# BadgerTechnologies/navigation

Hardware: AMD Instinct MI355X
Metric: scored trajectories/sec (whole node) + costmap inflation cells/sec, 400x400 map (higher is better)
Workload: dtype f64

## Files before the change

### navigation_amd/csrc/planner_bfs_rows.hip

```cpp
#include "planner_common.h"

namespace navgpu {

#ifdef NAVGPU_BFS_STATS
__device__ unsigned long long g_bfs_stats[16];
#define BFS_STAMP(v) const unsigned long long v = __builtin_amdgcn_s_memtime()
#define BFS_ACC(i, x) bst[i] += (x)
#else
#define BFS_STAMP(v)
#define BFS_ACC(i, x)
#endif
#ifndef NAVGPU_ROWS_RECORD_PAD
#define NAVGPU_ROWS_RECORD_PAD 4
#endif
constexpr uint32_t kRowsRecordPad = NAVGPU_ROWS_RECORD_PAD;
template <int W>
__host__ __device__ inline size_t bfs_rows_lds_words(uint32_t nx, uint32_t ny) {
  constexpr uint32_t Wp = (W + 3) & ~3u;
  const uint32_t nw = bfs_rows_waves(ny);
  return (((size_t)nw * kRowsPerWave * ((nx + 31) >> 5) + 3) & ~(size_t)3) + (size_t)kCareRows * kCareWords + (size_t)(nw + 2) * 2 * kRowsHalo * (2 * Wp + kRowsRecordPad);
}
__device__ __forceinline__ void rowsGroup4(const int g, const uint32_t aw, uint32_t& nz, uint32_t& lo, uint32_t& hi, uint32_t* __restrict__ b,
                                           uint32_t* __restrict__ f, const uint32_t L, const uint32_t R, uint32_t& p) {
  uint32_t u0, u1, u2, u3, t0, t1, t2, t3, st;
// ... 234 lines not shown
      BFS_ACC(7, aw != 0 ? 1 : 0);
      BFS_ACC(8, __builtin_popcount(aw));
      if (aw != 0) {
        uint32_t nz = 0, lo = 0, hi = 0;
        uint32_t p[2];
        const uint32_t zero = 0;
#pragma unroll
        for (int q = 0; q < NG; ++q)
          rowsGroup4(q, aw, nz, lo, hi, &blocked[4 * q], &fr[4 * q], q > 0 ? p[(q + 1) & 1] : zero, q + 1 < NG ? fr[q + 1 < NG ? 4 * q + 4 : 0] : zero,
                     p[q & 1]);
        BFS_STAMP(ts2);
        BFS_ACC(1, ts2 - ts1);
        if (wave_in_box && (nz & region_groups) != 0) {
#pragma unroll
          for (int q = 0; q < NG; ++q) {
            if (((nz & region_groups) >> q) & 1u) {
#pragma unroll
              for (int c = 0; c < 4; ++c) {
                const int j = 4 * q + c;
                if (j < W && j >= w0 && j <= w1) {
#ifndef NAVGPU_BFS_X_NOSTORE
                  if (row_in_box && fr[j < W ? j : 0] != 0) storeCells(j, fr[j < W ? j : 0], level + 1);
#endif
                }
              }
            }
          }
        }
        BFS_STAMP(ts3);
        BFS_ACC(2, ts3 - ts2);
        any_blk |= nz;
        a_own = (nz | (lo >> 1) | (hi << 1)) & gmask;
      }
      ++level;
    }
    BFS_STAMP(ts4);
    const uint32_t slot = xch % 3u;
    if (pub_top || pub_bot) {
#pragma unroll
      for (int q = 0; q < WP; q += 4) {
        *reinterpret_cast<uint4*>(edge + pub_wr + q) = make_uint4(fr[q], fr[q + 1], fr[q + 2], fr[q + 3]);
        *reinterpret_cast<uint4*>(edge + pub_wr + WP + q) = make_uint4(blocked[q], blocked[q + 1], blocked[q + 2], blocked[q + 3]);
      }
    }
    if (any_blk) s_flag[slot] = 1;
    if (wave_in_box) {
      uint32_t open_any = 0;
      const uint32_t rr = (uint32_t)(row_i - by0);
#pragma unroll
      for (int j = 0; j < W; ++j) {
        if (j >= w0 && j <= w1) {
          const uint32_t cw_i = (uint32_t)(j - w0);
          if (row_in_box) {
            const uint32_t care = (care_ok != 0 && cw_i < (uint32_t)kCareWords && rr < (uint32_t)kCareRows) ? care_l[rr * kCareWords + cw_i] : (care_ok ? 0u : 0xFFFFFFFFu);
            const int c_lo = max(bx0 - j * 32, 0), c_hi = min(bx1 - j * 32, 31);
            const uint32_t open = (~blocked[j] & care) | fr[j];
            if (c_hi >= c_lo) open_any |= open & (0xFFFFFFFFu >> (31 - c_hi)) & (0xFFFFFFFFu << c_lo);
          }
        }
      }
      if (open_any != 0) s_open[slot] = 1;
    }
    if (tid == 0) {
      s_flag[(xch + 1) % 3u] = 0;
      s_open[(xch + 1) % 3u] = 0;
    }
    BFS_STAMP(ts5);
    BFS_ACC(3, ts5 - ts4);
    __syncthreads();
    done = !s_flag[slot] || !s_open[slot];
    if (!done) {
      if ((halo_top || halo_bot) && real) {
#pragma unroll
        for (int q = 0; q < WP; q += 4) {
          const uint4 v = *reinterpret_cast<const uint4*>(edge + halo_rd + q);
          const uint4 b = *reinterpret_cast<const uint4*>(edge + halo_rd + WP + q);
          fr[q] = v.x;
          fr[q + 1] = v.y;
          fr[q + 2] = v.z;
          fr[q + 3] = v.w;
          blocked[q] = b.x;
          blocked[q + 1] = b.y;
          blocked[q + 2] = b.z;
          blocked[q + 3] = b.w;
        }
      }
      a_own = activity();
      __syncthreads();
    }
    ++xch;
    any_blk = 0;
    BFS_STAMP(ts6);
    BFS_ACC(4, ts6 - ts5);
  }
#ifdef NAVGPU_BFS_STATS
  if (lane == 0)
    for (int k = 0; k < 9; ++k) atomicAdd(&g_bfs_stats[k], bst[k]);
#endif
  if (pl.bfs_trace && tid == 0) pl.bfs_trace[(size_t)item * 8 + 3] = wall_clock64();

  __syncthreads();
  {
    uint32_t ex[WP], fb[WP];
#pragma unroll
    for (int j = 0; j < WP; ++j) {
      const bool in = owner && (uint32_t)j < Wr;
      fb[j] = in ? (freew[row * Wr + j] & ((uint32_t)j + 1 == Wr ? last_mask : 0xFFFFFFFFu)) : 0u;
      ex[j] = in ? ((blocked[j] & fb[j]) | seedm[row * Wr + j]) : 0u;
    }
    if (pub_top || pub_bot) {
#pragma unroll
      for (int j = 0; j < WP; ++j) edge[pub_wr + j] = ex[j];
    }
    __syncthreads();
    if ((halo_top || halo_bot) && real) {
#pragma unroll
      for (int j = 0; j < WP; ++j) ex[j] = edge[halo_rd + j];
    }
    if (wave_in_box) {
#pragma unroll
      for (int j = 0; j < W; ++j) {
        if (j >= w0 && j <= w1) {
          const uint32_t fc = ex[j];
          const uint32_t lw = j > 0 ? ex[j > 0 ? j - 1 : 0] : 0u, rw = j + 1 < WP ? ex[j + 1 < WP ? j + 1 : 0] : 0u;
          const uint32_t nbr = __builtin_amdgcn_alignbit(fc, lw, 31) | __builtin_amdgcn_alignbit(rw, fc, 1) | fromLaneBelow(fc) | fromLaneAbove(fc);
          const uint32_t cm = (uint32_t)j + 1 == Wr ? last_mask : ((uint32_t)j < Wr ? 0xFFFFFFFFu : 0u);
          const uint32_t touched = nbr & ~fb[j] & ~fc & cm;
          if (row_in_box) {
            storeCells(j, touched, N_obst);
            storeCells(j, ~fc & ~touched & cm, N_unreach);
          }
        }
      }
    }
  }
  if (pl.bfs_trace && tid == 0) {
    pl.bfs_trace[(size_t)item * 8 + 6] = wall_clock64();
    pl.bfs_trace[(size_t)item * 8 + 1] = wall_clock64() | ((unsigned long long)level << 48);
  }
  if (tid == 0 && pl.bfs_grids == 3) pl.bfs_levels[(size_t)inst * 3 + which] = level;
}
template <int W>
__global__ __launch_bounds__(1024, 6) void k_bfs_rows(PlannerDev pl, uint32_t first, uint32_t count, uint32_t* next_item, const uint32_t* order) {
  __shared__ uint32_t s_item;
  const uint32_t total = count * pl.bfs_grids;
  for (;;) {
    if (threadIdx.x == 0) s_item = atomicAdd(next_item, 1u);
    __syncthreads();
    const uint32_t slot = s_item;
    if (slot >= total) break;
    const uint32_t item = order ? order[slot] : slot;
    const uint32_t g = item / count;
    bfsRowsGrid<W>(pl, first + (item - g * count), (int)pl.bfs_grids - 1 - (int)g, item);
    __syncthreads();
  }
}
constexpr int kRows2HaloLanes = 4;
constexpr int kRows2Levels = 2 * kRows2HaloLanes;
constexpr int kRows2PerWave = 2 * (64 - 2 * kRows2HaloLanes);
constexpr int kRows2Words = 32;
__host__ __device__ inline uint32_t bfs_rows2_waves(uint32_t ny) { return (ny + kRows2PerWave - 1) / kRows2PerWave; }
__host__ __device__ inline size_t bfs_rows2_lds_words(uint32_t ny) {
  return (size_t)kCareRows * kCareWords + (size_t)(bfs_rows2_waves(ny) + 2) * 2 * kRows2HaloLanes * 4 * kRows2Words;
}
template <int G>
__device__ __forceinline__ void rows2Group(const uint32_t aw, uint32_t& nz, uint32_t& lo, uint32_t& hi, uint32_t* __restrict__ bA, uint32_t* __restrict__ bB,
                                           uint32_t* __restrict__ fA, uint32_t* __restrict__ fB, uint32_t& pA, uint32_t& pB, const uint32_t rA,
                                           const uint32_t rB) {
  uint32_t u0, u1, u2, u3, v0, v1, v2, v3, h0, h1, h2, h3, st;
#define NAVGPU_ROWS2_HEAD_FIRST                \
  "s_bitcmp1_b32 %[aw], %[g]\n\t"              \
  "s_cbranch_scc0 1f\n\t"                      \
  "v_lshlrev_b32 %[u0], 1, %[fA0]\n\t"         \
  "v_lshlrev_b32 %[v0], 1, %[fB0]\n\t"
#define NAVGPU_ROWS2_HEAD_NEXT                 \
  "s_bitcmp1_b32 %[aw], %[g]\n\t"              \
  "s_cbranch_scc0 1f\n\t"                      \
  "s_bitcmp1_b32 %[aw], %[gp]\n\t"             \
  "s_cbranch_scc1 3f\n\t"                      \
  "v_lshlrev_b32 %[u0], 1, %[fA0]\n\t"         \
  "v_lshlrev_b32 %[v0], 1, %[fB0]\n\t"         \
  "s_branch 4f\n\t"                            \
  "3:\n\t"                                     \
  "v_alignbit_b32 %[u0], %[fA0], %[pA], 31\n\t" \
  "v_alignbit_b32 %[v0], %[fB0], %[pB], 31\n\t" \
  "4:\n\t"
#define NAVGPU_ROWS2_BODY(HEAD)                                                                        \
  asm volatile(                                                                                        \
      HEAD                                                                                             \
      "v_alignbit_b32 %[u1], %[fA1], %[fA0], 31\n\t"                                                   \
      "v_alignbit_b32 %[u2], %[fA2], %[fA1], 31\n\t"                                                   \
      "v_alignbit_b32 %[u3], %[fA3], %[fA2], 31\n\t"                                                   \
      "v_alignbit_b32 %[v1], %[fB1], %[fB0], 31\n\t"                                                   \
      "v_alignbit_b32 %[v2], %[fB2], %[fB1], 31\n\t"                                                   \
      "v_alignbit_b32 %[v3], %[fB3], %[fB2], 31\n\t"                                                   \
      "v_mov_b32 %[pA], %[fA3]\n\t"                                                                    \
      "v_mov_b32 %[pB], %[fB3]\n\t"                                                                    \
      "v_alignbit_b32 %[h0], %[fA1], %[fA0], 1\n\t"                                                    \
      "v_alignbit_b32 %[h1], %[fA2], %[fA1], 1\n\t"                                                    \
      "v_alignbit_b32 %[h2], %[fA3], %[fA2], 1\n\t"                                                    \
      "v_alignbit_b32 %[h3], %[rA], %[fA3], 1\n\t"                                                     \
      "v_or_b32_dpp %[u0], %[fB0], %[u0] wave_shr:1 row_mask:0xf bank_mask:0xf bound_ctrl:1\n\t"       \
      "v_or_b32_dpp %[u1], %[fB1], %[u1] wave_shr:1 row_mask:0xf bank_mask:0xf bound_ctrl:1\n\t"       \
      "v_or_b32_dpp %[u2], %[fB2], %[u2] wave_shr:1 row_mask:0xf bank_mask:0xf bound_ctrl:1\n\t"       \
      "v_or_b32_dpp %[u3], %[fB3], %[u3] wave_shr:1 row_mask:0xf bank_mask:0xf bound_ctrl:1\n\t"       \
      "v_or3_b32 %[u0], %[u0], %[h0], %[fB0]\n\t"                                                      \
      "v_or3_b32 %[u1], %[u1], %[h1], %[fB1]\n\t"                                                      \
      "v_or3_b32 %[u2], %[u2], %[h2], %[fB2]\n\t"                                                      \
      "v_or3_b32 %[u3], %[u3], %[h3], %[fB3]\n\t"                                                      \
      "v_alignbit_b32 %[h0], %[fB1], %[fB0], 1\n\t"                                                    \
      "v_alignbit_b32 %[h1], %[fB2], %[fB1], 1\n\t"                                                    \
      "v_alignbit_b32 %[h2], %[fB3], %[fB2], 1\n\t"                                                    \
      "v_alignbit_b32 %[h3], %[rB], %[fB3], 1\n\t"                                                     \
      "v_or_b32_dpp %[v0], %[fA0], %[v0] wave_shl:1 row_mask:0xf bank_mask:0xf bound_ctrl:1\n\t"       \
      "v_or_b32_dpp %[v1], %[fA1], %[v1] wave_shl:1 row_mask:0xf bank_mask:0xf bound_ctrl:1\n\t"       \
      "v_or_b32_dpp %[v2], %[fA2], %[v2] wave_shl:1 row_mask:0xf bank_mask:0xf bound_ctrl:1\n\t"       \
      "v_or_b32_dpp %[v3], %[fA3], %[v3] wave_shl:1 row_mask:0xf bank_mask:0xf bound_ctrl:1\n\t"       \
      "v_or3_b32 %[v0], %[v0], %[h0], %[fA0]\n\t"                                                      \
      "v_or3_b32 %[v1], %[v1], %[h1], %[fA1]\n\t"                                                      \
      "v_or3_b32 %[v2], %[v2], %[h2], %[fA2]\n\t"                                                      \
      "v_or3_b32 %[v3], %[v3], %[h3], %[fA3]\n\t"                                                      \
      "v_bitop3_b32 %[fA0], %[u0], %[bA0], %[u0] bitop3:0x30\n\t"                                      \
      "v_bitop3_b32 %[fA1], %[u1], %[bA1], %[u1] bitop3:0x30\n\t"                                      \
      "v_bitop3_b32 %[fA2], %[u2], %[bA2], %[u2] bitop3:0x30\n\t"                                      \
      "v_bitop3_b32 %[fA3], %[u3], %[bA3], %[u3] bitop3:0x30\n\t"                                      \
      "v_bitop3_b32 %[fB0], %[v0], %[bB0], %[v0] bitop3:0x30\n\t"                                      \
      "v_bitop3_b32 %[fB1], %[v1], %[bB1], %[v1] bitop3:0x30\n\t"                                      \
      "v_bitop3_b32 %[fB2], %[v2], %[bB2], %[v2] bitop3:0x30\n\t"                                      \
      "v_bitop3_b32 %[fB3], %[v3], %[bB3], %[v3] bitop3:0x30\n\t"                                      \
      "v_or_b32_e32 %[bA0], %[bA0], %[u0]\n\t"                                                         \
      "v_or_b32_e32 %[bA1], %[bA1], %[u1]\n\t"                                                         \
      "v_or_b32_e32 %[bA2], %[bA2], %[u2]\n\t"                                                         \
      "v_or_b32_e32 %[bA3], %[bA3], %[u3]\n\t"                                                         \
      "v_or_b32_e32 %[bB0], %[bB0], %[v0]\n\t"                                                         \
      "v_or_b32_e32 %[bB1], %[bB1], %[v1]\n\t"                                                         \
      "v_or_b32_e32 %[bB2], %[bB2], %[v2]\n\t"                                                         \
      "v_or_b32_e32 %[bB3], %[bB3], %[v3]\n\t"                                                         \
      "v_or_b32_e32 %[h0], %[fA0], %[fB0]\n\t"                                                         \
      "v_or_b32_e32 %[h3], %[fA3], %[fB3]\n\t"                                                         \
      "v_or3_b32 %[h1], %[fA1], %[fA2], %[fB1]\n\t"                                                    \
      "v_or3_b32 %[h2], %[h0], %[h3], %[fB2]\n\t"                                                      \
      "v_or_b32_e32 %[h1], %[h1], %[h2]\n\t"                                                           \
      "v_cmp_ne_u32_e32 vcc, 0, %[h1]\n\t"                                                             \
      "s_cbranch_vccz 1f\n\t"                                                                          \
      "s_bitset1_b32 %[nz], %[g]\n\t"                                                                  \
      "v_cmp_ne_u32_e32 vcc, 0, %[h0]\n\t"                                                             \
      "s_cbranch_vccz 3f\n\t"                                                                          \
      "s_bitset1_b32 %[lo], %[g]\n\t"                                                                  \
      "3:\n\t"                                                                                         \
      "v_cmp_ne_u32_e32 vcc, 0, %[h3]\n\t"                                                             \
      "s_cbranch_vccz 1f\n\t"                                                                          \
      "s_bitset1_b32 %[hi], %[g]\n\t"                                                                  \
      "1:\n\t"                                                                                         \
      : [bA0] "+v"(bA[0]), [bA1] "+v"(bA[1]), [bA2] "+v"(bA[2]), [bA3] "+v"(bA[3]), [bB0] "+v"(bB[0]), [bB1] "+v"(bB[1]), [bB2] "+v"(bB[2]),  \
        [bB3] "+v"(bB[3]), [fA0] "+v"(fA[0]), [fA1] "+v"(fA[1]), [fA2] "+v"(fA[2]), [fA3] "+v"(fA[3]), [fB0] "+v"(fB[0]), [fB1] "+v"(fB[1]),   \
        [fB2] "+v"(fB[2]), [fB3] "+v"(fB[3]), [pA] "+v"(pA), [pB] "+v"(pB), [nz] "+s"(nz), [lo] "+s"(lo), [hi] "+s"(hi), [u0] "=&v"(u0),       \
        [u1] "=&v"(u1), [u2] "=&v"(u2), [u3] "=&v"(u3), [v0] "=&v"(v0), [v1] "=&v"(v1), [v2] "=&v"(v2), [v3] "=&v"(v3), [h0] "=&v"(h0),        \
        [h1] "=&v"(h1), [h2] "=&v"(h2), [h3] "=&v"(h3), [st] "=&s"(st)                                                                         \
      : [aw] "s"(aw), [g] "n"(G), [gp] "n"(G > 0 ? G - 1 : 0), [rA] "v"(rA), [rB] "v"(rB)                                                      \
      : "vcc", "scc")
  if constexpr (G == 0) NAVGPU_ROWS2_BODY(NAVGPU_ROWS2_HEAD_FIRST);
  else NAVGPU_ROWS2_BODY(NAVGPU_ROWS2_HEAD_NEXT);
#undef NAVGPU_ROWS2_BODY
#undef NAVGPU_ROWS2_HEAD_FIRST
#undef NAVGPU_ROWS2_HEAD_NEXT
}
template <int G>
__device__ __forceinline__ void rows2Level(const uint32_t aw, uint32_t& nz, uint32_t& lo, uint32_t& hi, uint32_t* __restrict__ blA, uint32_t* __restrict__ blB,
                                           uint32_t* __restrict__ frA, uint32_t* __restrict__ frB, uint32_t& pA, uint32_t& pB, const uint32_t zero) {
  constexpr int NG = kRows2Words / 4;
  if constexpr (G < NG) {
    rows2Group<G>(aw, nz, lo, hi, blA + 4 * G, blB + 4 * G, frA + 4 * G, frB + 4 * G, pA, pB, G + 1 < NG ? frA[G + 1 < NG ? 4 * G + 4 : 0] : zero,
                  G + 1 < NG ? frB[G + 1 < NG ? 4 * G + 4 : 0] : zero);
    rows2Level<G + 1>(aw, nz, lo, hi, blA, blB, frA, frB, pA, pB, zero);
  }
}
__device__ __forceinline__ void bfsRows2Grid(const PlannerDev& pl, const uint32_t inst, const int which, const uint32_t item, uint32_t* seedw) {
  constexpr int W = kRows2Words, NG = W / 4, D = kRows2Levels, HL = kRows2HaloLanes;
  int bx0 = 0, bx1 = -1, by0 = 0, by1 = -1, care_ok = 0;
  if (pl.bfs_bounded) {
    const int4 bb = reinterpret_cast<const int4*>(pl.bfs_box)[2 * inst];
    bx0 = __builtin_amdgcn_readfirstlane(bb.x);
    bx1 = __builtin_amdgcn_readfirstlane(bb.y);
    by0 = __builtin_amdgcn_readfirstlane(bb.z);
    by1 = __builtin_amdgcn_readfirstlane(bb.w);
    care_ok = __builtin_amdgcn_readfirstlane(pl.bfs_box[8 * inst + 4]);
  }
  if (!(bx1 >= bx0 && by1 >= by0)) {
    bx0 = 0;
    by0 = 0;
    bx1 = (int)pl.nx - 1;
    by1 = (int)pl.ny - 1;
    care_ok = 0;
  }
  extern __shared__ __align__(16) uint32_t sm[];
  __shared__ uint32_t s_wave[16];
  __shared__ uint32_t s_flag[3];
  __shared__ uint32_t s_open[3];
  uint32_t tid_ = threadIdx.x, nx_ = pl.nx, ny_ = pl.ny;
  asm volatile("" : "+v"(tid_), "+s"(nx_), "+s"(ny_));
  const uint32_t tid = tid_;
  if (pl.bfs_trace && tid == 0) pl.bfs_trace[(size_t)item * 8] = wall_clock64();
  const Geom g = geomOf(pl, inst);
  const uint32_t nx = nx_, ny = ny_, Wr = (nx + 31) >> 5;
  const uint32_t nw = blockDim.x >> 6;
  const uint32_t lane = tid & 63u, wave_id = tid >> 6;
// ... 174 lines not shown
    if (any_blk) s_flag[slot] = 1;
    if (wave_in_box) {
      uint32_t open_any = 0;
      const uint32_t rrA = (uint32_t)(rowA_i - by0), rrB = (uint32_t)(rowB_i - by0);
#pragma unroll
      for (int j = 0; j < W; ++j) {
        if (j >= w0 && j <= w1) {
          const uint32_t cw_i = (uint32_t)(j - w0);
          const int c_lo = max(bx0 - j * 32, 0), c_hi = min(bx1 - j * 32, 31);
          const uint32_t cm = c_hi >= c_lo ? ((0xFFFFFFFFu >> (31 - c_hi)) & (0xFFFFFFFFu << c_lo)) : 0u;
          if (inA) {
            const uint32_t care = (care_ok != 0 && cw_i < (uint32_t)kCareWords && rrA < (uint32_t)kCareRows) ? care_l[rrA * kCareWords + cw_i] : (care_ok ? 0u : 0xFFFFFFFFu);
            open_any |= ((~blA[j] & care) | frA[j]) & cm;
          }
          if (inB) {
            const uint32_t care = (care_ok != 0 && cw_i < (uint32_t)kCareWords && rrB < (uint32_t)kCareRows) ? care_l[rrB * kCareWords + cw_i] : (care_ok ? 0u : 0xFFFFFFFFu);
            open_any |= ((~blB[j] & care) | frB[j]) & cm;
          }
        }
      }
      if (open_any != 0) s_open[slot] = 1;
    }
    if (tid == 0) {
      s_flag[(xch + 1) % 3u] = 0;
      s_open[(xch + 1) % 3u] = 0;
    }
    BFS_STAMP(ts5);
    BFS_ACC(3, ts5 - ts4);
    __syncthreads();
    done = !s_flag[slot] || !s_open[slot];
    if (!done) {
      if (halo_top || halo_bot) {
#pragma unroll
        for (int q = 0; q < W; q += 4) {
          if (realA) {
            unquad(*reinterpret_cast<const uint4*>(edge + halo_rd + q), frA + q);
            unquad(*reinterpret_cast<const uint4*>(edge + halo_rd + W + q), blA + q);
          }
          if (realB) {
            unquad(*reinterpret_cast<const uint4*>(edge + halo_rd + 2 * W + q), frB + q);
            unquad(*reinterpret_cast<const uint4*>(edge + halo_rd + 3 * W + q), blB + q);
          }
        }
      }
      a_own = activity();
      __syncthreads();
    }
    ++xch;
    any_blk = 0;
    BFS_STAMP(ts6);
    BFS_ACC(4, ts6 - ts5);
  }
#ifdef NAVGPU_BFS_STATS
  if (lane == 0)
    for (int k = 0; k < 9; ++k) atomicAdd(&g_bfs_stats[k], bst[k]);
#endif
  if (pl.bfs_trace && tid == 0) pl.bfs_trace[(size_t)item * 8 + 3] = wall_clock64();

  __syncthreads();
  {
#pragma unroll
    for (int q = 0; q < NG; ++q) {
      const uint4 sA = ownerA ? rowWords(seedw, rowA, q) : make_uint4(0, 0, 0, 0), sB = ownerB ? rowWords(seedw, rowB, q) : make_uint4(0, 0, 0, 0);
      const uint4 fA = ownerA ? rowWords(freew, rowA, q) : make_uint4(0, 0, 0, 0), fB = ownerB ? rowWords(freew, rowB, q) : make_uint4(0, 0, 0, 0);
      const uint32_t sa[4] = {sA.x, sA.y, sA.z, sA.w}, sb[4] = {sB.x, sB.y, sB.z, sB.w}, fa[4] = {fA.x, fA.y, fA.z, fA.w}, fb[4] = {fB.x, fB.y, fB.z, fB.w};
#pragma unroll
      for (int c = 0; c < 4; ++c) {
        const int j = 4 * q + c;
        const bool in = (uint32_t)j < Wr;
        blA[j] = (in && ownerA) ? ((blA[j] & fa[c] & colMask(j)) | sa[c]) : 0u;
        blB[j] = (in && ownerB) ? ((blB[j] & fb[c] & colMask(j)) | sb[c]) : 0u;
      }
    }
    if (lane == (uint32_t)HL || lane == 63u - HL) {
      const bool top = lane == (uint32_t)HL;
      uint32_t* rec = edge + ((wave_id + 1) * 2 + (top ? 0u : 1u)) * HL * 4 * W;
#pragma unroll
      for (int j = 0; j < W; ++j) rec[j] = top ? blA[j] : blB[j];
    }
    __syncthreads();
    if (lane == (uint32_t)HL - 1u && realB) {
      const uint32_t* rec = edge + (wave_id * 2 + 1) * HL * 4 * W;
#pragma unroll
      for (int j = 0; j < W; ++j) blB[j] = rec[j];
    }
    if (lane == 64u - HL && realA) {
      const uint32_t* rec = edge + ((wave_id + 2) * 2) * HL * 4 * W;
#pragma unroll
      for (int j = 0; j < W; ++j) blA[j] = rec[j];
    }
    if (wave_in_box) {
#pragma unroll
      for (int j = 0; j < W; ++j) {
        if (j >= w0 && j <= w1) {
          const uint32_t cm = (uint32_t)j + 1 == Wr ? last_mask : ((uint32_t)j < Wr ? 0xFFFFFFFFu : 0u);
          const uint32_t eA = blA[j], eB = blB[j];
          const uint32_t lA = j > 0 ? blA[j > 0 ? j - 1 : 0] : 0u, rA = j + 1 < W ? blA[j + 1 < W ? j + 1 : 0] : 0u;
          const uint32_t lB = j > 0 ? blB[j > 0 ? j - 1 : 0] : 0u, rB = j + 1 < W ? blB[j + 1 < W ? j + 1 : 0] : 0u;
          const uint32_t upA = fromLaneBelow(eB), dnB = fromLaneAbove(eA);
          if (inA) {
            const uint32_t nbr = __builtin_amdgcn_alignbit(eA, lA, 31) | __builtin_amdgcn_alignbit(rA, eA, 1) | upA | eB;
            const uint32_t fb = freew[rowA * Wr + j] & cm;
            const uint32_t touched = nbr & ~fb & ~eA & cm;
            storeCells(rowA, j, touched, N_obst);
            storeCells(rowA, j, ~eA & ~touched & cm, N_unreach);
          }
          if (inB) {
            const uint32_t nbr = __builtin_amdgcn_alignbit(eB, lB, 31) | __builtin_amdgcn_alignbit(rB, eB, 1) | eA | dnB;
            const uint32_t fb = freew[rowB * Wr + j] & cm;
            const uint32_t touched = nbr & ~fb & ~eB & cm;
            storeCells(rowB, j, touched, N_obst);
            storeCells(rowB, j, ~eB & ~touched & cm, N_unreach);
          }
        }
      }
    }
  }
  if (pl.bfs_trace && tid == 0) {
    pl.bfs_trace[(size_t)item * 8 + 6] = wall_clock64();
    pl.bfs_trace[(size_t)item * 8 + 1] = wall_clock64() | ((unsigned long long)level << 48);
  }
  if (tid == 0 && pl.bfs_grids == 3) pl.bfs_levels[(size_t)inst * 3 + which] = level;
}
__global__ __launch_bounds__(768, 3) void k_bfs_rows2(PlannerDev pl, uint32_t first, uint32_t count, uint32_t* next_item, const uint32_t* order, uint32_t* scratch) {
  __shared__ uint32_t s_item;
  const uint32_t total = count * pl.bfs_grids;
  uint32_t* seedw = scratch + (size_t)blockIdx.x * pl.ny * ((pl.nx + 31) >> 5);
  for (;;) {
    if (threadIdx.x == 0) s_item = atomicAdd(next_item, 1u);
    __syncthreads();
    const uint32_t slot = s_item;
    if (slot >= total) break;
    const uint32_t item = order ? order[slot] : slot;
    const uint32_t g = item / count;
    bfsRows2Grid(pl, first + (item - g * count), (int)pl.bfs_grids - 1 - (int)g, item, seedw);
    __syncthreads();
  }
}
static int bfs_rows_words(uint32_t nx, uint32_t ny) {
  if (NAVGPU_DEBUG_ENV("NAVGPU_DEBUG_BFS_NO_ROWS")) return 0;
  const uint32_t Wr = (nx + 31) / 32;
  if (bfs_rows_waves(ny) > 16) return 0;
  return Wr <= 7 ? 7 : (Wr <= 13 ? 13 : (Wr <= 20 ? 20 : 0));
}
bool bfs_rows_fits(uint32_t nx, uint32_t ny) { return bfs_rows_words(nx, ny) != 0; }
template <int W>
static void launch_bfs_rows_w(const PlannerDev& pl, uint32_t first, uint32_t count, hipStream_t s, const uint32_t* order) {
  const uint32_t nw = bfs_rows_waves(pl.ny);
  const size_t lds = bfs_rows_lds_words<W>(pl.nx, pl.ny) * 4;
  if (lds > 48 * 1024) hipFuncSetAttribute((const void*)k_bfs_rows<W>, hipFuncAttributeMaxDynamicSharedMemorySize, (int)lds);
  const uint32_t per_cu = std::max<uint32_t>(1u, std::min<uint32_t>(std::min<uint32_t>(24u / nw, (uint32_t)((156u * 1024u) / (lds + 1024))), 4u));
  hipLaunchKernelGGL(k_bfs_rows<W>, dim3(std::min(count * pl.bfs_grids, per_cu * bfs_cu_count())), dim3(nw * 64), lds, s, pl, first, count, pl.bfs_next_item + 1, order);
}
bool launch_bfs_rows(const PlannerDev& pl, uint32_t first, uint32_t count, hipStream_t s, const uint32_t* order) {
  switch (bfs_rows_words(pl.nx, pl.ny)) {
    case 7: launch_bfs_rows_w<7>(pl, first, count, s, order); return true;
    case 13: launch_bfs_rows_w<13>(pl, first, count, s, order); return true;
    case 20: launch_bfs_rows_w<20>(pl, first, count, s, order); return true;
    default: return false;
  }
}
bool launch_bfs_rows2(const PlannerDev& pl, uint32_t first, uint32_t count, hipStream_t s, const uint32_t* order) {
  if (NAVGPU_DEBUG_ENV("NAVGPU_DEBUG_BFS_NO_ROWS")) return false;
  if ((pl.nx + 31) / 32 > (uint32_t)kRows2Words || bfs_rows2_waves(pl.ny) > 12) return false;
  const size_t lds2 = bfs_rows2_lds_words(pl.ny) * 4;
  if (lds2 > 48 * 1024) hipFuncSetAttribute((const void*)k_bfs_rows2, hipFuncAttributeMaxDynamicSharedMemorySize, (int)lds2);
  hipLaunchKernelGGL(k_bfs_rows2, dim3(std::min(count * pl.bfs_grids, bfs_cu_count())), dim3(bfs_rows2_waves(pl.ny) * 64), lds2, s, pl, first, count, pl.bfs_next_item, order, pl.bfs_scratch);
  return true;
}

#ifdef NAVGPU_BFS_STATS
extern "C" int navgpu_debug_bfs_stats(unsigned long long* out16, int reset) {
  if (out16) hipMemcpyFromSymbol(out16, HIP_SYMBOL(g_bfs_stats), sizeof(unsigned long long) * 16);
  if (reset) {
    unsigned long long z[16] = {0};
    hipMemcpyToSymbol(HIP_SYMBOL(g_bfs_stats), z, sizeof(z));
  }
  return 0;
}
#endif

}
```

Baseline: 5.641 billion.

## Add column-split row BFS variant using two waves per row block

New measurement: 5.399 billion. 0.957x the previous value.

```diff
diff --git a/navigation_amd/csrc/planner_bfs_rows.hip b/navigation_amd/csrc/planner_bfs_rows.hip
--- a/navigation_amd/csrc/planner_bfs_rows.hip
+++ b/navigation_amd/csrc/planner_bfs_rows.hip
@@ -410,6 +410,343 @@
     const uint32_t item = order ? order[slot] : slot;
     const uint32_t g = item / count;
     bfsRowsGrid<W>(pl, first + (item - g * count), (int)pl.bfs_grids - 1 - (int)g, item);
+    __syncthreads();
+  }
+}
+constexpr int kRowsSplitCut = 7;
+constexpr int kRowsSplitWords = 8;
+#ifndef NAVGPU_ROWS_SPLIT_HALO
+#define NAVGPU_ROWS_SPLIT_HALO 7
+#endif
+constexpr int kRowsSplitHalo = NAVGPU_ROWS_SPLIT_HALO;
+constexpr int kRowsSplitPerWave = 64 - 2 * kRowsSplitHalo;
+constexpr uint32_t kRowsSplitRecord = 2 * kRowsSplitWords + kRowsRecordPad;
+__host__ __device__ inline uint32_t bfs_rows_split_blocks(uint32_t ny) { return (ny + kRowsSplitPerWave - 1) / kRowsSplitPerWave; }
+__host__ __device__ inline size_t bfs_rows_split_lds_words(uint32_t nx, uint32_t ny) {
+  const uint32_t nb = bfs_rows_split_blocks(ny);
+  return (((size_t)nb * kRowsSplitPerWave * ((nx + 31) >> 5) + 3) & ~(size_t)3) + (size_t)kCareRows * kCareWords +
+         (size_t)(nb + 2) * 2 * 2 * kRowsSplitHalo * kRowsSplitRecord + (size_t)nb * 2 * 64 * 2;
+}
+template <int W>
+__device__ __forceinline__ void bfsRowsSplitGrid(const PlannerDev& pl, const uint32_t inst, const int which, const uint32_t item) {
+  constexpr int CUT = kRowsSplitCut, WP = kRowsSplitWords, NG = WP / 4, D = kRowsSplitHalo, RPW = kRowsSplitPerWave;
+  static_assert(W > CUT && CUT + 1 <= WP && W - CUT + 1 <= WP, "either half and its halo word fit the lane's words");
+  int bx0 = 0, bx1 = -1, by0 = 0, by1 = -1, care_ok = 0;
+  if (pl.bfs_bounded) {
+    const int4 bb = reinterpret_cast<const int4*>(pl.bfs_box)[2 * inst];
+    bx0 = __builtin_amdgcn_readfirstlane(bb.x);
+    bx1 = __builtin_amdgcn_readfirstlane(bb.y);
+    by0 = __builtin_amdgcn_readfirstlane(bb.z);
+    by1 = __builtin_amdgcn_readfirstlane(bb.w);
+    care_ok = __builtin_amdgcn_readfirstlane(pl.bfs_box[8 * inst + 4]);
+  }
+  if (!(bx1 >= bx0 && by1 >= by0)) {
+    bx0 = 0;
+    by0 = 0;
+    bx1 = (int)pl.nx - 1;
+    by1 = (int)pl.ny - 1;
+    care_ok = 0;
+  }
+  extern __shared__ __align__(16) uint32_t sm[];
+  __shared__ uint32_t s_wave[16];
+  __shared__ uint32_t s_flag[3];
+  __shared__ uint32_t s_open[3];
+  uint32_t tid_ = threadIdx.x, nx_ = pl.nx, ny_ = pl.ny;
+  asm volatile("" : "+v"(tid_), "+s"(nx_), "+s"(ny_));
+  const uint32_t tid = tid_;
+  if (pl.bfs_trace && tid == 0) pl.bfs_trace[(size_t)item * 8] = wall_clock64();
+  const Geom g = geomOf(pl, inst);
+  const uint32_t nx = nx_, ny = ny_, Wr = (nx + 31) >> 5;
+  const uint32_t nb = blockDim.x >> 7;
+  const uint32_t lane = tid & 63u, wave_id = (uint32_t)__builtin_amdgcn_readfirstlane((int)(tid >> 6));
+  const uint32_t rb = wave_id >> 1, half = wave_id & 1u;
+  const int off = half ? CUT - 1 : 0;
+  const int row_i = (int)(rb * RPW + lane) - D;
+  const bool real = row_i >= 0 && row_i < (int)ny;
+  const bool owner = real && lane >= (uint32_t)D && lane < 64u - D;
+  const uint32_t row = real ? (uint32_t)row_i : 0u;
+  const uint32_t rows_p = nb * RPW;
+  const uint32_t seed_words = (rows_p * Wr + 3u) & ~3u;
+  constexpr uint32_t RS = kRowsSplitRecord;
+  uint32_t* seedm = sm;
+  uint32_t* care_l = sm + seed_words;
+  uint32_t* edge = care_l + kCareRows * kCareWords;
+  const uint32_t edge_words = (nb + 2) * 2 * 2 * D * RS;
+  uint32_t* cut = edge + edge_words;
+  const uint32_t cut_words = nb * 2 * 64 * 2;
+  const uint8_t* master = pl.master + (size_t)inst * pl.cells_padded;
+  const uint32_t* freew = bfsFreeBitmap(pl, which, inst, ny * Wr);
+  uint32_t* dist = (which == 0 ? pl.path : (which == 1 ? pl.goal : pl.goal_front)) + (size_t)inst * pl.cells;
+  const uint32_t N_obst = pl.cells, N_unreach = pl.cells + 1;
+  const uint32_t last_mask = (nx & 31) ? ((1u << (nx & 31)) - 1u) : 0xFFFFFFFFu;
+  const bool aligned4 = (nx & 3) == 0;
+
+  for (uint32_t i = tid; i < seed_words + kCareRows * kCareWords + edge_words + cut_words; i += blockDim.x) sm[i] = 0;
+  if (tid < 3) s_flag[tid] = s_open[tid] = 0;
+  __syncthreads();
+  if (pl.bfs_trace && tid == 0) pl.bfs_trace[(size_t)item * 8 + 4] = wall_clock64();
+  if (care_ok) {
+    const uint32_t* care = pl.bfs_care + (size_t)inst * kCareRows * kCareWords;
+    for (uint32_t i = tid; i < (uint32_t)(kCareRows * kCareWords); i += blockDim.x) care_l[i] = care[i];
+  }
+  rowsPlanSeeds(pl, inst, which, g, master, nx, tid, s_wave, [&](uint32_t mx, uint32_t my) {
+    atomicOr(&seedm[my * Wr + (mx >> 5)], 1u << (mx & 31));
+  });
+  __syncthreads();
+  if (pl.bfs_trace && tid == 0) pl.bfs_trace[(size_t)item * 8 + 5] = wall_clock64();
+
+  const uint32_t* freer = freew + row * Wr + off;
+  const uint32_t* seedr = seedm + row * Wr + off;
+  uint32_t blocked[WP], fr[WP];
+#pragma unroll
+  for (int j = 0; j < WP; ++j) {
+    blocked[j] = 0xFFFFFFFFu;
+    fr[j] = 0;
+    if (real && (uint32_t)(j + off) < Wr) {
+      fr[j] = seedr[j];
+      blocked[j] = ~(freer[j] & ((uint32_t)(j + off) + 1 == Wr ? last_mask : 0xFFFFFFFFu)) | fr[j];
+    }
+  }
+  const int lw0 = max(bx0 >> 5, half ? CUT : 0) - off, lw1 = min(min(bx1 >> 5, half ? W - 1 : CUT - 1), (int)Wr - 1) - off;
+  const bool wave_in_box = (int)(rb * RPW) <= by1 && (int)((rb + 1) * RPW) > by0 && lw1 >= lw0;
+  const bool row_in_box = owner && row_i >= by0 && row_i <= by1;
+  const int cw0 = off - (bx0 >> 5);
+  uint32_t region_groups = 0;
+  for (int jr = lw0; jr <= lw1; ++jr) region_groups |= 1u << (jr >> 2);
+  uint32_t* drow = dist + (size_t)row * nx + off * 32;
+  auto storeCells = [&](int j, uint32_t cells, uint32_t value) {
+    uint32_t* dw = drow + j * 32;
+    if (aligned4) {
+      uint32_t full = cells & (cells >> 1) & (cells >> 2) & (cells >> 3) & 0x11111111u;
+      cells &= ~(full * 15u);
+      const uint4 v4 = make_uint4(value, value, value, value);
+      while (full) {
+        const uint32_t bpos = (uint32_t)__ffs(full) - 1u;
+        *reinterpret_cast<uint4*>(dw + bpos) = v4;
+        full &= full - 1;
+      }
+    }
+    while (cells) {
+      const uint32_t bpos = (uint32_t)__ffs(cells) - 1u;
+      dw[bpos] = value;
+      cells &= cells - 1;
+    }
+  };
+  auto vrec = [&](uint32_t slot, uint32_t h, uint32_t bottom) { return ((slot * 2 + h) * 2 + bottom) * D; };
+  const bool pub_top = lane >= (uint32_t)D && lane < 2u * D, pub_bot = lane >= 64u - 2 * D && lane < 64u - D;
+  const uint32_t pub_wr = (vrec(rb + 1, half, pub_top ? 0u : 1u) + (pub_top ? lane - D : lane - (64u - 2 * D))) * RS;
+  const bool halo_top = lane < (uint32_t)D, halo_bot = lane >= 64u - D;
+  const uint32_t halo_row = halo_top ? lane : lane - (64u - D);
+  const uint32_t halo_rd = (vrec(halo_top ? rb : rb + 2, half, halo_top ? 1u : 0u) + halo_row) * RS;
+  const uint32_t corner_rd = (vrec(halo_top ? rb : rb + 2, half ^ 1u, halo_top ? 1u : 0u) + halo_row) * RS + (half ? CUT - 1 : 1);
+  const uint32_t cut_wr = (wave_id * 64 + lane) * 2, cut_rd = ((wave_id ^ 1u) * 64 + lane) * 2;
+  constexpr uint32_t gmask = (1u << NG) - 1u;
+
+  auto activity = [&]() -> uint32_t {
+    uint32_t nz = 0, lo = 0, hi = 0;
+#pragma unroll
+    for (int q = 0; q < NG; ++q) {
+      const uint32_t t = fr[4 * q] | fr[4 * q + 1] | fr[4 * q + 2] | fr[4 * q + 3];
+      if (__builtin_amdgcn_ballot_w64(t != 0) != 0) {
+        nz |= 1u << q;
+        if (__builtin_amdgcn_ballot_w64(fr[4 * q] != 0) != 0) lo |= 1u << q;
+        if (__builtin_amdgcn_ballot_w64(fr[4 * q + 3] != 0) != 0) hi |= 1u << q;
+      }
+    }
+    return (nz | (lo >> 1) | (hi << 1)) & gmask;
+  };
+  if (wave_in_box) {
+    uint32_t seed_dist = 0;
+    asm volatile("" : "+s"(seed_dist));
+#pragma unroll
+    for (int j = 0; j < WP; ++j)
+      if (j >= lw0 && j <= lw1 && row_in_box) storeCells(j, fr[j], seed_dist);
+  }
+  uint32_t a_own = activity();
+  uint32_t level = 0, xch = 0, any_blk = 0;
+  if (pl.bfs_trace && tid == 0) pl.bfs_trace[(size_t)item * 8 + 2] = wall_clock64();
+  bool done = false;
+#ifdef NAVGPU_BFS_STATS
+  unsigned long long bst[9] = {0, 0, 0, 0, 0, 0, 0, 0, 0};
+#endif
+  while (!done) {
+    for (int k = 0; k < D; ++k) {
+      BFS_STAMP(ts1);
+      BFS_ACC(5, 1);
+      const uint32_t aw = __builtin_amdgcn_readfirstlane(a_own);
+      BFS_ACC(7, aw != 0 ? 1 : 0);
+      BFS_ACC(8, __builtin_popcount(aw));
+      if (aw != 0) {
+        uint32_t nz = 0, lo = 0, hi = 0;
+        uint32_t p[2];
+        const uint32_t zero = 0;
+        rowsGroup4(0, aw, nz, lo, hi, &blocked[0], &fr[0], zero, fr[4], p[0]);
+        rowsGroup4(1, aw, nz, lo, hi, &blocked[4], &fr[4], p[0], zero, p[1]);
+        BFS_STAMP(ts2);
+        BFS_ACC(1, ts2 - ts1);
+        if (wave_in_box && (nz & region_groups) != 0) {
+#pragma unroll
+          for (int q = 0; q < NG; ++q) {
+            if (((nz & region_groups) >> q) & 1u) {
+#pragma unroll
+              for (int c = 0; c < 4; ++c) {
+                const int j = 4 * q + c;
+                if (j >= lw0 && j <= lw1) {
+                  if (row_in_box && fr[j] != 0) storeCells(j, fr[j], level + 1);
+                }
+              }
+            }
+          }
+        }
+        BFS_STAMP(ts3);
+        BFS_ACC(2, ts3 - ts2);
+        any_blk |= nz;
+        a_own = (nz | (lo >> 1) | (hi << 1)) & gmask;
+      }
+      ++level;
+    }
+    BFS_STAMP(ts4);
+    const uint32_t slot = xch % 3u;
+    if (pub_top || pub_bot) {
+#pragma unroll
+      for (int q = 0; q < WP; q += 4) {
+        *reinterpret_cast<uint4*>(edge + pub_wr + q) = make_uint4(fr[q], fr[q + 1], fr[q + 2], fr[q + 3]);
+        *reinterpret_cast<uint4*>(edge + pub_wr + WP + q) = make_uint4(blocked[q], blocked[q + 1], blocked[q + 2], blocked[q + 3]);
+      }
+    }
+    *reinterpret_cast<uint2*>(cut + cut_wr) = half ? make_uint2(fr[1], blocked[1]) : make_uint2(fr[CUT - 1], blocked[CUT - 1]);
+    if (any_blk) s_flag[slot] = 1;
+    if (wave_in_box) {
+      uint32_t open_any = 0;
+      const uint32_t rr = (uint32_t)(row_i - by0);
+#pragma unroll
+      for (int j = 0; j < WP; ++j) {
+        if (j >= lw0 && j <= lw1) {
+          const uint32_t cw_i = (uint32_t)(j + cw0);
+          if (row_in_box) {
+            const uint32_t care = (care_ok != 0 && cw_i < (uint32_t)kCareWords && rr < (uint32_t)kCareRows) ? care_l[rr * kCareWords + cw_i] : (care_ok ? 0u : 0xFFFFFFFFu);
+            const int c_lo = max(bx0 - (j + off) * 32, 0), c_hi = min(bx1 - (j + off) * 32, 31);
+            const uint32_t open = (~blocked[j] & care) | fr[j];
+            if (c_hi >= c_lo) open_any |= open & (0xFFFFFFFFu >> (31 - c_hi)) & (0xFFFFFFFFu << c_lo);
+          }
+        }
+      }
+      if (open_any != 0) s_open[slot] = 1;
+    }
+    if (tid == 0) {
+      s_flag[(xch + 1) % 3u] = 0;
+      s_open[(xch + 1) % 3u] = 0;
+    }
+    BFS_STAMP(ts5);
+    BFS_ACC(3, ts5 - ts4);
+    __syncthreads();
+    done = !s_flag[slot] || !s_open[slot];
+    if (!done) {
+      uint32_t hf, hb;
+      if (halo_top || halo_bot) {
+        if (real) {
+#pragma unroll
+          for (int q = 0; q < WP; q += 4) {
+            const uint4 v = *reinterpret_cast<const uint4*>(edge + halo_rd + q);
+            const uint4 b = *reinterpret_cast<const uint4*>(edge + halo_rd + WP + q);
+            fr[q] = v.x;
+            fr[q + 1] = v.y;
+            fr[q + 2] = v.z;
+            fr[q + 3] = v.w;
+            blocked[q] = b.x;
+            blocked[q + 1] = b.y;
+            blocked[q + 2] = b.z;
+            blocked[q + 3] = b.w;
+          }
+        }
+        hf = edge[corner_rd];
+        hb = edge[corner_rd + WP];
+      } else {
+        const uint2 c = *reinterpret_cast<const uint2*>(cut + cut_rd);
+        hf = c.x;
+        hb = c.y;
+      }
+      if (real) {
+        if (half) {
+          fr[0] = hf;
+          blocked[0] = hb;
+        } else {
+          fr[CUT] = hf;
+          blocked[CUT] = hb;
+        }
+      }
+      a_own = activity();
+      __syncthreads();
+    }
+    ++xch;
+    any_blk = 0;
+    BFS_STAMP(ts6);
+    BFS_ACC(4, ts6 - ts5);
+  }
+#ifdef NAVGPU_BFS_STATS
+  if (lane == 0)
+    for (int k = 0; k < 9; ++k) atomicAdd(&g_bfs_stats[k], bst[k]);
+#endif
+  if (pl.bfs_trace && tid == 0) pl.bfs_trace[(size_t)item * 8 + 3] = wall_clock64();
+
+  __syncthreads();
+  {
+    uint32_t ex[WP], fb[WP];
+#pragma unroll
+    for (int j = 0; j < WP; ++j) {
+      const bool in = owner && j >= (half ? 1 : 0) && j < (half ? WP : CUT) && (uint32_t)(j + off) < Wr;
+      fb[j] = in ? (freer[j] & ((uint32_t)(j + off) + 1 == Wr ? last_mask : 0xFFFFFFFFu)) : 0u;
+      ex[j] = in ? ((blocked[j] & fb[j]) | seedr[j]) : 0u;
+    }
+    if (pub_top || pub_bot) {
+#pragma unroll
+      for (int j = 0; j < WP; ++j) edge[pub_wr + j] = ex[j];
+    }
+    cut[cut_wr] = half ? ex[1] : ex[CUT - 1];
+    __syncthreads();
+    if ((halo_top || halo_bot) && real) {
+#pragma unroll
+      for (int j = 0; j < WP; ++j) ex[j] = edge[halo_rd + j];
+    } else if (!(halo_top || halo_bot)) {
+      const uint32_t c = cut[cut_rd];
+      if (half) ex[0] = c;
+      else ex[CUT] = c;
+    }
+    if (wave_in_box) {
+#pragma unroll
+      for (int j = 0; j < WP; ++j) {
+        if (j >= lw0 && j <= lw1) {
+          const uint32_t fc = ex[j];
+          const uint32_t lw = j > 0 ? ex[j > 0 ? j - 1 : 0] : 0u, rw = j + 1 < WP ? ex[j + 1 < WP ? j + 1 : 0] : 0u;
+          const uint32_t nbr = __builtin_amdgcn_alignbit(fc, lw, 31) | __builtin_amdgcn_alignbit(rw, fc, 1) | fromLaneBelow(fc) | fromLaneAbove(fc);
+          const uint32_t cm = (uint32_t)(j + off) + 1 == Wr ? last_mask : 0xFFFFFFFFu;
+          const uint32_t touched = nbr & ~fb[j] & ~fc & cm;
+          if (row_in_box) {
+            storeCells(j, touched, N_obst);
+            storeCells(j, ~fc & ~touched & cm, N_unreach);
+          }
+        }
+      }
+    }
+  }
+  if (pl.bfs_trace && tid == 0) {
+    pl.bfs_trace[(size_t)item * 8 + 6] = wall_clock64();
+    pl.bfs_trace[(size_t)item * 8 + 1] = wall_clock64() | ((unsigned long long)level << 48);
+  }
+  if (tid == 0 && pl.bfs_grids == 3) pl.bfs_levels[(size_t)inst * 3 + which] = level;
+}
+template <int W>
+__global__ __launch_bounds__(1024, 8) void k_bfs_rows_split(PlannerDev pl, uint32_t first, uint32_t count, uint32_t* next_item, const uint32_t* order) {
+  __shared__ uint32_t s_item;
+  const uint32_t total = count * pl.bfs_grids;
+  for (;;) {
+    if (threadIdx.x == 0) s_item = atomicAdd(next_item, 1u);
+    __syncthreads();
+    const uint32_t slot = s_item;
+    if (slot >= total) break;
+    const uint32_t item = order ? order[slot] : slot;
+    const uint32_t g = item / count;
+    bfsRowsSplitGrid<W>(pl, first + (item - g * count), (int)pl.bfs_grids - 1 - (int)g, item);
     __syncthreads();
   }
 }
@@ -890,10 +1227,27 @@
   const uint32_t per_cu = std::max<uint32_t>(1u, std::min<uint32_t>(std::min<uint32_t>(24u / nw, (uint32_t)((156u * 1024u) / (lds + 1024))), 4u));
   hipLaunchKernelGGL(k_bfs_rows<W>, dim3(std::min(count * pl.bfs_grids, per_cu * bfs_cu_count())), dim3(nw * 64), lds, s, pl, first, count, pl.bfs_next_item + 1, order);
 }
+constexpr uint32_t kRowsSplitSlotShareNum = 1, kRowsSplitSlotShareDen = 2;
+static bool bfs_rows_split_takes(const PlannerDev& pl, uint32_t count) {
+  const uint32_t Wr = (pl.nx + 31) / 32, nb = bfs_rows_split_blocks(pl.ny);
+  if (Wr <= (uint32_t)kRowsSplitCut || nb > 8) return false;
+  if (const char* e = NAVGPU_DEBUG_ENV("NAVGPU_DEBUG_BFS_SPLIT")) return e[0] != '0';
+  return (uint64_t)count * pl.bfs_grids * 2 * nb * kRowsSplitSlotShareDen <= (uint64_t)bfs_cu_count() * 32 * kRowsSplitSlotShareNum;
+}
+static void launch_bfs_rows_split13(const PlannerDev& pl, uint32_t first, uint32_t count, hipStream_t s, const uint32_t* order) {
+  const uint32_t nb = bfs_rows_split_blocks(pl.ny);
+  const size_t lds = bfs_rows_split_lds_words(pl.nx, pl.ny) * 4;
+  if (lds > 48 * 1024) hipFuncSetAttribute((const void*)k_bfs_rows_split<13>, hipFuncAttributeMaxDynamicSharedMemorySize, (int)lds);
+  const uint32_t per_cu = std::max<uint32_t>(1u, std::min<uint32_t>(std::min<uint32_t>(16u / nb, (uint32_t)((156u * 1024u) / (lds + 1024))), 4u));
+  hipLaunchKernelGGL(k_bfs_rows_split<13>, dim3(std::min(count * pl.bfs_grids, per_cu * bfs_cu_count())), dim3(nb * 128), lds, s, pl, first, count, pl.bfs_next_item + 1, order);
+}
 bool launch_bfs_rows(const PlannerDev& pl, uint32_t first, uint32_t count, hipStream_t s, const uint32_t* order) {
   switch (bfs_rows_words(pl.nx, pl.ny)) {
     case 7: launch_bfs_rows_w<7>(pl, first, count, s, order); return true;
-    case 13: launch_bfs_rows_w<13>(pl, first, count, s, order); return true;
+    case 13:
+      if (bfs_rows_split_takes(pl, count)) launch_bfs_rows_split13(pl, first, count, s, order);
+      else launch_bfs_rows_w<13>(pl, first, count, s, order);
+      return true;
     case 20: launch_bfs_rows_w<20>(pl, first, count, s, order); return true;
     default: return false;
   }
```
